# calclavia/tal-asrd

Hardware: AMD Instinct MI355X
Metric: audio frames/sec (16 kHz, 10 ms hop) end-to-end log-mel -> TDS encoder -> diarization head (higher is better)
Workload: dtype f32 (dense layers: 3 x f16 MFMA hi/lo split, f32 accumulate); 1 GPU; 1 x 3600 s 16 kHz clip per GPU, each a whole-episode B=1 call (BASELINE.json configs[2]; SDModel path of tal/baseline/reconcile.py:76-85: log-mel -> TDS 80-800-1120-1440 -> 128-d feat + argmax over 6008 speakers); weights=synthetic deterministic, audio_resident_in_hbm=True

## Files before the change

tal_asrd_amd/csrc/gemm_common.h:

```cpp
#pragma once
#include "common.h"

namespace tal {

constexpr int BK = 32;

template <int MODE, int NSUB>
__device__ __forceinline__ void gemm_epilogue(const GemmArgs& g, const f32x16 (&acc)[NSUB], float* lds, float* Y,
                                              const float* bias, const float* res, int64_t m0, int n0, int lane,
                                              int w, int wm, int wn) {
    const int64_t M = g.M;
    const int N = g.N;
    const int colb = lane & 31;
    const int rowb = 4 * (lane >> 5);
    const float alpha = g.alpha;
    const f32x4 zero4 = {0.f, 0.f, 0.f, 0.f};
    float amax = 0.f;
    constexpr int CW = 32 * NSUB;
    if (MODE == 4) {
        float bcol[NSUB];
#pragma unroll
        for (int j = 0; j < NSUB; ++j) {
            const int col = n0 + (wn * NSUB + j) * 32 + colb;
            bcol[j] = (bias && col < N) ? bias[col] : 0.f;
// ... 38 lines not shown
        const bool cols_full = n_base + CW <= N;
        const bool buf_ok = g.ldy < (1 << 21) && (MODE != 2 || g.ldres < (1 << 21));
        auto uptr = [](const float* p) {
            const uint64_t v = reinterpret_cast<uint64_t>(p);
            const uint32_t lo = __builtin_amdgcn_readfirstlane((uint32_t)v), hi = __builtin_amdgcn_readfirstlane((uint32_t)(v >> 32));
            return reinterpret_cast<void*>(((uint64_t)hi << 32) | lo);
        };
        __amdgpu_buffer_rsrc_t rs_y[2], rs_res[2];
#pragma unroll
        for (int half = 0; half < 2; ++half) {
            const int64_t row0 = m0 + wm * 32 + half * 16;
            const int rows_valid = (int)(M - row0 < 0 ? 0 : (M - row0 > 16 ? 16 : M - row0));
            const int ext_y = rows_valid > 0 ? (int)(((rows_valid - 1) * g.ldy + CW) * 4) : 0;
            const int ext_r = rows_valid > 0 && MODE == 2 ? (int)(((rows_valid - 1) * g.ldres + CW) * 4) : 0;
            rs_y[half] = __builtin_amdgcn_make_buffer_rsrc(uptr(Y + row0 * g.ldy + n_base), 0, __builtin_amdgcn_readfirstlane(ext_y), 0x00020000);
            rs_res[half] = __builtin_amdgcn_make_buffer_rsrc(uptr(MODE == 2 ? res + row0 * g.ldres + n_base : Y), 0,
                                                             __builtin_amdgcn_readfirstlane(ext_r), 0x00020000);
        }
        __amdgpu_buffer_rsrc_t rs_bias = __builtin_amdgcn_make_buffer_rsrc(uptr(bias ? bias + n_base : Y), 0, CW * 4, 0x00020000);
#pragma unroll
        for (int half = 0; half < 2; ++half) {
#pragma unroll
            for (int j = 0; j < NSUB; ++j)
#pragma unroll
                for (int e8 = 0; e8 < 8; ++e8) {
                    const int e = half * 8 + e8;
                    const int r = rowb + (e8 & 3) + 8 * (e8 >> 2);
                    stage[r * CW + j * 32 + colb] = acc[j][e];
                }
            if (cols_full && buf_ok) {
                typedef unsigned u32x4 __attribute__((ext_vector_type(4)));
                int r = lane / (CW / 4), c4 = lane - r * (CW / 4);
                int offy[2 * NSUB], offr[2 * NSUB], offb[2 * NSUB], ldsv[2 * NSUB];
                f32x4 rv[2 * NSUB], bv[2 * NSUB];
#pragma unroll
                for (int t = 0; t < 2 * NSUB; ++t) {
                    offy[t] = (r * (int)g.ldy + c4 * 4) * 4;
                    offr[t] = (r * (int)g.ldres + c4 * 4) * 4;
                    offb[t] = c4 * 16;
                    ldsv[t] = r * CW + c4 * 4;
                    c4 += 64 - CW / 4;
                    r += 1;
                    if (c4 >= CW / 4) {
                        c4 -= CW / 4;
                        r += 1;
                    }
                }
                typedef unsigned u32x2r __attribute__((ext_vector_type(2)));
                u32x2r rh[2 * NSUB], rl[2 * NSUB];
#pragma unroll
                for (int t = 0; t < 2 * NSUB; ++t) {
                    if (MODE == 2 && g.res_split) {
                        const int cw = offb[t] >> 2;
                        const int so = offr[t] - offb[t] + (cw >> 5) * 128 + (cw & 31) * 2;
                        rh[t] = __builtin_amdgcn_raw_buffer_load_b64(rs_res[half], so, 0, 0);
                        rl[t] = __builtin_amdgcn_raw_buffer_load_b64(rs_res[half], so + 64, 0, 0);
                    } else if (MODE == 2)
                        rv[t] = __builtin_bit_cast(f32x4, __builtin_amdgcn_raw_buffer_load_b128(rs_res[half], offr[t], 0, 0));
                    bv[t] = bias ? __builtin_bit_cast(f32x4, __builtin_amdgcn_raw_buffer_load_b128(rs_bias, offb[t], 0, 0)) : zero4;
                }
#pragma unroll
                for (int t = 0; t < 2 * NSUB; ++t) {
                    f32x4 v = *reinterpret_cast<const f32x4*>(&stage[ldsv[t]]) + bv[t];
                    if (MODE == 1) {
                        v.x = fmaxf(v.x, 0.f); v.y = fmaxf(v.y, 0.f); v.z = fmaxf(v.z, 0.f); v.w = fmaxf(v.w, 0.f);
                    }
                    if (MODE == 2 && g.res_split) {
                        const f16x4 h4 = __builtin_bit_cast(f16x4, rh[t]), l4 = __builtin_bit_cast(f16x4, rl[t]);
#pragma unroll
                        for (int q = 0; q < 4; ++q) rv[t][q] = (float)h4[q] + (float)l4[q] * (1.0f / 2048.0f);
                    }
                    if (MODE == 2) v = rv[t] + alpha * v;
                    if (MODE == 3 && (g.scale_cols == 0 || n_base + (offb[t] >> 2) < g.scale_cols)) v = alpha * v;
                    if (g.out_split) {
                        typedef unsigned u32x2 __attribute__((ext_vector_type(2)));
                        f16x4 hi, lo;
                        amax = amax4(amax, v);
                        if (g.range_flag) {
                            f16x2p h01, l01, h23, l23;
                            split_f16x3_pair(v.x, v.y, h01, l01);
                            split_f16x3_pair(v.z, v.w, h23, l23);
                            hi = {h01[0], h01[1], h23[0], h23[1]};
                            lo = {l01[0], l01[1], l23[0], l23[1]};
                        } else {
#pragma unroll
                            for (int q = 0; q < 4; ++q) {
                                _Float16 h, l;
                                split_f16x3(v[q], h, l);
                                hi[q] = h;
                                lo[q] = l;
                            }
                        }
                        const int cw = offb[t] >> 2;
                        const int so = offy[t] - offb[t] + (cw >> 5) * 128 + (cw & 31) * 2;
                        __builtin_amdgcn_raw_buffer_store_b64(__builtin_bit_cast(u32x2, hi), rs_y[half], so, 0, 0);
                        __builtin_amdgcn_raw_buffer_store_b64(__builtin_bit_cast(u32x2, lo), rs_y[half], so + 64, 0, 0);
                        continue;
                    }
                    __builtin_amdgcn_raw_buffer_store_b128(__builtin_bit_cast(u32x4, v), rs_y[half], offy[t], 0, 0);
                }
                if (g.out_split && half == 1) note_range(amax, g.range_flag);
                continue;
            }
#pragma unroll
            for (int t = 0; t < 2 * NSUB; ++t) {
                const int i = lane + 64 * t;
                const int r = i / (CW / 4);
                const int c = (i - r * (CW / 4)) * 4;
                const int64_t row = m0 + wm * 32 + half * 16 + r;
                const int col = n_base + c;
                if (row < M && col < N) {
                    f32x4 v = *reinterpret_cast<const f32x4*>(&stage[r * CW + c]);
                    if (col + 3 < N) {
                        if (bias) v += *reinterpret_cast<const f32x4*>(bias + col);
                        if (MODE == 1) {
                            v.x = fmaxf(v.x, 0.f); v.y = fmaxf(v.y, 0.f); v.z = fmaxf(v.z, 0.f); v.w = fmaxf(v.w, 0.f);
                        }
                        if (MODE == 2) v = *reinterpret_cast<const f32x4*>(res + row * g.ldres + col) + alpha * v;
                        if (MODE == 3 && (g.scale_cols == 0 || col < g.scale_cols)) v = alpha * v;
                        *reinterpret_cast<f32x4*>(Y + row * g.ldy + col) = v;
                    } else {
                        for (int q = 0; q < 4 && col + q < N; ++q) {
                            float x = v[q] + (bias ? bias[col + q] : 0.f);
                            if (MODE == 1) x = fmaxf(x, 0.f);
                            if (MODE == 2) x = res[row * g.ldres + col + q] + alpha * x;
                            if (MODE == 3 && (g.scale_cols == 0 || col + q < g.scale_cols)) x = alpha * x;
                            Y[row * g.ldy + col + q] = x;
                        }
                    }
                }
            }
        }
    } else {
#pragma unroll
        for (int j = 0; j < NSUB; ++j) {
            const int col = n0 + (wn * NSUB + j) * 32 + colb;
            if (col >= N) continue;
            const float bv = bias ? bias[col] : 0.f;
#pragma unroll
            for (int e = 0; e < 16; ++e) {
                const int64_t row = m0 + wm * 32 + rowb + (e & 3) + 8 * (e >> 2);
                if (row < M) {
                    float v = acc[j][e] + bv;
                    if (MODE == 1) v = fmaxf(v, 0.f);
                    if (MODE == 2) v = res[row * g.ldres + col] + alpha * v;
                    if (MODE == 3 && (g.scale_cols == 0 || col < g.scale_cols)) v = alpha * v;
                    Y[row * g.ldy + col] = v;
                }
            }
        }
    }
}

template <int MODE, int NSUB>
__device__ __forceinline__ void gemm_epilogue_split(const GemmArgs& g, const f32x16 (&acc)[NSUB], float* lds, float* Y,
                                                    const float* res, int64_t m0, int n0, int lane, int w) {
    static_assert(MODE == 1 || MODE == 2, "relu or residual");
    constexpr int CW = 32 * NSUB;
    typedef unsigned u32x2 __attribute__((ext_vector_type(2)));
    typedef float f32x2 __attribute__((ext_vector_type(2)));
    const int64_t M = g.M;
    const int colb = lane & 31, rowb = 4 * (lane >> 5);
    float* stage = lds + w * (16 * CW);
    auto uptr = [](const float* p) {
        const uint64_t v = reinterpret_cast<uint64_t>(p);
        const uint32_t lo = __builtin_amdgcn_readfirstlane((uint32_t)v), hi = __builtin_amdgcn_readfirstlane((uint32_t)(v >> 32));
        return reinterpret_cast<void*>(((uint64_t)hi << 32) | lo);
    };
    const int lr = lane >> 3, lp = lane & 7;
    const int ldy4 = (int)g.ldy * 4, ldr4 = (int)g.ldres * 4;
    const int vy0 = lr * ldy4 + lp * 8, vy1 = vy0 + 8 * ldy4;
    const int vr0 = lr * ldr4 + lp * 8, vr1 = vr0 + 8 * ldr4;
    const float* sp = stage + lr * CW + lp * 4;
    const float alpha = g.alpha;
    const f32x2 al2 = {alpha, alpha}, s11 = {1.0f / 2048.0f, 1.0f / 2048.0f};
    float amax = 0.f;
#pragma unroll
    for (int half = 0; half < 2; ++half) {
        const int64_t row0 = m0 + w * 32 + half * 16;
        const int rows_valid = (int)(M - row0 < 0 ? 0 : (M - row0 > 16 ? 16 : M - row0));
        const int ext_y = rows_valid > 0 ? (rows_valid - 1) * ldy4 + CW * 4 : 0;
        const int ext_r = rows_valid > 0 && MODE == 2 ? (rows_valid - 1) * ldr4 + CW * 4 : 0;
        __amdgpu_buffer_rsrc_t rs_y = __builtin_amdgcn_make_buffer_rsrc(uptr(Y + row0 * g.ldy + n0), 0, __builtin_amdgcn_readfirstlane(ext_y), 0x00020000);
        __amdgpu_buffer_rsrc_t rs_r = __builtin_amdgcn_make_buffer_rsrc(uptr(MODE == 2 ? res + row0 * g.ldres + n0 : Y), 0,
                                                                      __builtin_amdgcn_readfirstlane(ext_r), 0x00020000);
        u32x2 rh[2 * NSUB], rl[2 * NSUB];
        if (MODE == 2) {
#pragma unroll
            for (int t = 0; t < 2 * NSUB; ++t) {
                const int rg = t / NSUB, b = t % NSUB;
                rh[t] = __builtin_amdgcn_raw_buffer_load_b64(rs_r, (rg ? vr1 : vr0) + b * 128, 0, 0);
                rl[t] = __builtin_amdgcn_raw_buffer_load_b64(rs_r, (rg ? vr1 : vr0) + b * 128 + 64, 0, 0);
            }
        }
#pragma unroll
        for (int j = 0; j < NSUB; ++j)
#pragma unroll
            for (int e8 = 0; e8 < 8; ++e8) {
                const int r = rowb + (e8 & 3) + 8 * (e8 >> 2);
                stage[r * CW + j * 32 + colb] = acc[j][half * 8 + e8];
            }
        f32x4 sv[2 * NSUB];
#pragma unroll
        for (int t = 0; t < 2 * NSUB; ++t) sv[t] = *reinterpret_cast<const f32x4*>(sp + (t / NSUB) * 8 * CW + (t % NSUB) * 32);
#pragma unroll
        for (int t = 0; t < 2 * NSUB; ++t) {
            const int rg = t / NSUB, b = t % NSUB;
            f32x2 va = {sv[t][0], sv[t][1]}, vb = {sv[t][2], sv[t][3]};
            if (MODE == 1) {
                va = __builtin_elementwise_max(va, f32x2{0.f, 0.f});
                vb = __builtin_elementwise_max(vb, f32x2{0.f, 0.f});
            } else {
                const f16x4 h4 = __builtin_bit_cast(f16x4, rh[t]), l4 = __builtin_bit_cast(f16x4, rl[t]);
                const f32x2 ha = {(float)h4[0], (float)h4[1]}, hb = {(float)h4[2], (float)h4[3]};
                const f32x2 la = {(float)l4[0], (float)l4[1]}, lb = {(float)l4[2], (float)l4[3]};
                va = al2 * va + (la * s11 + ha);
                vb = al2 * vb + (lb * s11 + hb);
            }
            amax = __builtin_fmaxf(amax, __builtin_fmaxf(__builtin_fabsf(va[0]), __builtin_fabsf(va[1])));
            amax = __builtin_fmaxf(amax, __builtin_fmaxf(__builtin_fabsf(vb[0]), __builtin_fabsf(vb[1])));
            f16x2p h01, l01, h23, l23;
            split_f16x3_pair(va[0], va[1], h01, l01);
            split_f16x3_pair(vb[0], vb[1], h23, l23);
            const f16x4 hi = {h01[0], h01[1], h23[0], h23[1]}, lo = {l01[0], l01[1], l23[0], l23[1]};
            __builtin_amdgcn_raw_buffer_store_b64(__builtin_bit_cast(u32x2, hi), rs_y, (rg ? vy1 : vy0) + b * 128, 0, 0);
            __builtin_amdgcn_raw_buffer_store_b64(__builtin_bit_cast(u32x2, lo), rs_y, (rg ? vy1 : vy0) + b * 128 + 64, 0, 0);
        }
    }
    note_range(amax, g.range_flag);
}

__device__ __forceinline__ unsigned logical_tile_of(unsigned nb, unsigned bid) {
    const unsigned xcd = bid & 7u, q = nb >> 3, r = nb & 7u;
    return (xcd < r ? xcd * (q + 1) : r * (q + 1) + (xcd - r) * q) + (bid >> 3);
}
__device__ __forceinline__ unsigned logical_tile() { return logical_tile_of(gridDim.x, blockIdx.x); }

}
```

tal_asrd_amd/csrc/gemm_f32.hip:

```cpp
#include "gemm_common.h"

namespace tal {

template <int MODE, int NSUB, bool SPLITK, int STAGE, bool F16X3 = false, int EPI = 0>
__global__ __launch_bounds__(256, F16X3 ? 2 : 1) void gemm_glds_kernel(const GemmArgs g) {
    __builtin_amdgcn_s_setprio(3);
    constexpr int BM = 128, BN = 32 * NSUB;
    constexpr int ROWS = BM + BN;
    constexpr int CHUNKS = ROWS / 8;
    constexpr int PER_WAVE = CHUNKS / 4;
    __shared__ __attribute__((aligned(16))) float lds[2 * ROWS * 32];

    const bool is_slice = SPLITK && blockIdx.x >= (unsigned)g.tile_base;
    const unsigned sbid = blockIdx.x - (unsigned)g.tile_base;
    const int slice = is_slice ? (int)(sbid / (unsigned)g.tail_tiles) : 0;
    const unsigned logical = is_slice ? (unsigned)g.tile_base + sbid % (unsigned)g.tail_tiles
                                      : (SPLITK ? logical_tile_of((unsigned)g.tile_base, blockIdx.x) : logical_tile());
    const unsigned tile_m = g.tiles_n == 1 ? logical : __umulhi(logical, g.tiles_n_magic);
    const int64_t m0 = (int64_t)tile_m * BM;
    const int n0 = (int)(logical - tile_m * (unsigned)g.tiles_n) * BN;
    const int64_t M = g.M;
    const int N = g.N, K = g.K;
    const int z1 = EPI ? 0 : (int)blockIdx.y / g.nb2, z2 = EPI ? 0 : (int)blockIdx.y % g.nb2;
    const float* A = g.A + z1 * g.a_s1 + z2 * g.a_s2;
    const float* W = g.W + z1 * g.w_s1 + z2 * g.w_s2;
    float* Y = g.Y + z1 * g.y_s1 + z2 * g.y_s2;
    const float* bias = g.bias ? g.bias + z2 * g.bias_s2 : nullptr;
    const float* res = g.res ? g.res + z1 * g.r_s1 + z2 * g.r_s2 : nullptr;

    const int tid = threadIdx.x;
    const int lane = tid & 63;
    const int w = wave_id();
    const int wm = w, wn = 0;

    const int sub = lane >> 3;
    const int srccol = ((lane & 7) ^ (((w & 1) * 4 + (lane >> 4)) & 7)) * 4;
    const int a_rows = (int)((M - m0) < BM ? (M - m0) : BM) - 1;
    const int b_rows = ((N - n0) < BN ? (N - n0) : BN) - 1;
    const float* src[PER_WAVE];
#pragma unroll
    for (int t = 0; t < PER_WAVE; ++t) {
        const int row = 8 * (w + 4 * t) + sub;
        if (t < 4)
            src[t] = A + (m0 + min(row, a_rows)) * g.lda + srccol;
        else
            src[t] = W + (int64_t)(n0 + min(row - BM, b_rows)) * g.ldw + srccol;
    }
    auto uniform_ptr = [](const float* p) {
        const uint64_t v = reinterpret_cast<uint64_t>(p);
        const uint32_t lo = __builtin_amdgcn_readfirstlane((uint32_t)v), hi = __builtin_amdgcn_readfirstlane((uint32_t)(v >> 32));
        return reinterpret_cast<void*>(((uint64_t)hi << 32) | lo);
    };
    __amdgpu_buffer_rsrc_t rsrc_a = __builtin_amdgcn_make_buffer_rsrc(uniform_ptr(A + m0 * g.lda), 0, 0x7fffffff, 0x00020000);
    __amdgpu_buffer_rsrc_t rsrc_w = __builtin_amdgcn_make_buffer_rsrc(uniform_ptr(W + (int64_t)n0 * g.ldw), 0, 0x7fffffff, 0x00020000);
    int voff[PER_WAVE];
#pragma unroll
    for (int t = 0; t < PER_WAVE; ++t) {
        const int row = 8 * (w + 4 * t) + sub;
        voff[t] = t < 4 ? (int)((min(row, a_rows) * g.lda + srccol) * 4) : (int)((min(row - BM, b_rows) * g.ldw + srccol) * 4);
    }
    auto issue = [&](int kt, int buf) {
#pragma unroll
        for (int t = 0; t < PER_WAVE; ++t) {
            float* dst = lds + buf * (ROWS * 32) + (w + 4 * t) * 256;
            if (STAGE == 2) {
#if defined(__HIP_DEVICE_COMPILE__)
                __builtin_amdgcn_raw_ptr_buffer_load_lds(t < 4 ? rsrc_a : rsrc_w, (__attribute__((address_space(3))) void*)dst, 16,
                                                         voff[t], kt * (BK * 4), 0, 0);
#endif
            } else
                __builtin_amdgcn_global_load_lds((const __attribute__((address_space(1))) void*)(src[t] + kt * BK),
                                                 (__attribute__((address_space(3))) void*)dst, 16, 0, 0);
        }
    };

    f32x16 acc[NSUB];
    f32x16 accx[F16X3 ? NSUB : 1];
#pragma unroll
    for (int j = 0; j < NSUB; ++j) {
        const float b0 = (EPI && bias && !is_slice) ? bias[n0 + j * 32 + (lane & 31)] : 0.f;
#pragma unroll
        for (int e = 0; e < 16; ++e) acc[j][e] = b0;
    }
#pragma unroll
    for (int j = 0; j < (F16X3 ? NSUB : 1); ++j)
#pragma unroll
        for (int e = 0; e < 16; ++e) accx[j][e] = 0.f;

    const int frow = lane & 31;
    const int fsw = (frow >> 1) & 7;
    const int fhalf = lane >> 5;
    const int nk_all = K / BK;
    const int kt0 = is_slice ? (int)((int64_t)slice * nk_all / g.split) : 0;
    const int nk = is_slice ? (int)((int64_t)(slice + 1) * nk_all / g.split) : nk_all;
    issue(kt0, kt0 & 1);
    __builtin_amdgcn_s_setprio(0);
    __builtin_assume(kt0 < nk);
    for (int kt = kt0; kt < nk; ++kt) {
        asm volatile("s_waitcnt vmcnt(0)" ::: "memory");
        __syncthreads();
        if (kt + 1 < nk) issue(kt + 1, (kt + 1) & 1);
        const float* As = lds + (kt & 1) * (ROWS * 32) + (wm * 32 + frow) * 32;
        const float* Bs = lds + (kt & 1) * (ROWS * 32) + (BM + frow) * 32;
        if (F16X3) {
            f16x8 ahi[2], alo[2], bhi[3], blo[3];
            auto slh = [&](int gk) { return ((2 * gk + fhalf) ^ fsw) * 4; };
            auto sll = [&](int gk) { return ((4 + 2 * gk + fhalf) ^ fsw) * 4; };
            auto read_b = [&](int q, int slot) {
                const int gk = q / NSUB, j = q % NSUB;
                bhi[slot] = *reinterpret_cast<const f16x8*>(Bs + j * 32 * 32 + slh(gk));
                blo[slot] = *reinterpret_cast<const f16x8*>(Bs + j * 32 * 32 + sll(gk));
            };
            ahi[0] = *reinterpret_cast<const f16x8*>(As + slh(0));
            alo[0] = *reinterpret_cast<const f16x8*>(As + sll(0));
            read_b(0, 0);
            read_b(1, 1);
#pragma unroll
            for (int q = 0; q < 2 * NSUB; ++q) {
                const int gk = q / NSUB, j = q % NSUB;
                if (q + 2 < 2 * NSUB) read_b(q + 2, (q + 2) % 3);
                if (q == NSUB - 2) {
                    ahi[1] = *reinterpret_cast<const f16x8*>(As + slh(1));
                    alo[1] = *reinterpret_cast<const f16x8*>(As + sll(1));
                }
                __builtin_amdgcn_sched_barrier(0);
                acc[j] = __builtin_amdgcn_mfma_f32_32x32x16_f16(ahi[gk], bhi[q % 3], acc[j], 0, 0, 0);
                accx[F16X3 ? j : 0] = __builtin_amdgcn_mfma_f32_32x32x16_f16(ahi[gk], blo[q % 3], accx[F16X3 ? j : 0], 0, 0, 0);
                accx[F16X3 ? j : 0] = __builtin_amdgcn_mfma_f32_32x32x16_f16(alo[gk], bhi[q % 3], accx[F16X3 ? j : 0], 0, 0, 0);
                __builtin_amdgcn_sched_barrier(0);
            }
            continue;
        }
        f32x4 fa[2], fb[2][NSUB];
        fa[0] = *reinterpret_cast<const f32x4*>(As + ((fhalf) ^ fsw) * 4);
#pragma unroll
        for (int j = 0; j < NSUB; ++j) fb[0][j] = *reinterpret_cast<const f32x4*>(Bs + j * 32 * 32 + ((fhalf) ^ fsw) * 4);
#pragma unroll
        for (int kk = 0; kk < BK / 8; ++kk) {
            const int cur = kk & 1, nxt = cur ^ 1;
            if (kk + 1 < BK / 8) {
                const int sl = ((2 * (kk + 1) + fhalf) ^ fsw) * 4;
                fa[nxt] = *reinterpret_cast<const f32x4*>(As + sl);
#pragma unroll
                for (int j = 0; j < NSUB; ++j) fb[nxt][j] = *reinterpret_cast<const f32x4*>(Bs + j * 32 * 32 + sl);
            }
#pragma unroll
            for (int j = 0; j < NSUB; ++j) {
                acc[j] = __builtin_amdgcn_mfma_f32_32x32x2f32(fa[cur].x, fb[cur][j].x, acc[j], 0, 0, 0);
                acc[j] = __builtin_amdgcn_mfma_f32_32x32x2f32(fa[cur].y, fb[cur][j].y, acc[j], 0, 0, 0);
                acc[j] = __builtin_amdgcn_mfma_f32_32x32x2f32(fa[cur].z, fb[cur][j].z, acc[j], 0, 0, 0);
                acc[j] = __builtin_amdgcn_mfma_f32_32x32x2f32(fa[cur].w, fb[cur][j].w, acc[j], 0, 0, 0);
            }
        }
    }
    asm volatile("s_waitcnt vmcnt(0)" ::: "memory");
    __syncthreads();
    __builtin_amdgcn_s_setprio(3);
    if (F16X3) {
        typedef float f32x2 __attribute__((ext_vector_type(2)));
        const f32x2 s11 = {1.0f / 2048.0f, 1.0f / 2048.0f};
#pragma unroll
        for (int j = 0; j < NSUB; ++j)
#pragma unroll
            for (int e = 0; e < 16; e += 2) {
                const f32x2 x2 = {accx[F16X3 ? j : 0][e], accx[F16X3 ? j : 0][e + 1]}, a2 = {acc[j][e], acc[j][e + 1]};
                const f32x2 o2 = __builtin_elementwise_fma(x2, s11, a2);
                acc[j][e] = o2[0];
                acc[j][e + 1] = o2[1];
            }
    }
    if (is_slice) {
        GemmArgs gp = g;
        gp.M = m0 + BM;
        gp.N = n0 + BN;
        gp.ldy = BN;
        gp.out_split = 0;
        float* tile_ws = g.splitk_ws + ((size_t)(logical - g.tile_base) * g.split + slice) * (BM * BN);
        gemm_epilogue<0, NSUB>(gp, acc, lds, tile_ws - (m0 * BN + n0), nullptr, nullptr, m0, n0, lane, w, wm, wn);
    } else {
        if constexpr (EPI != 0) gemm_epilogue_split<MODE, NSUB>(g, acc, lds, Y, res, m0, n0, lane, w);
        else gemm_epilogue<MODE, NSUB>(g, acc, lds, Y, bias, res, m0, n0, lane, w, wm, wn);
    }
}

template <int MODE, int WAVES_M, int NSUB, int BKT>
__global__ __launch_bounds__(256) void gemm_nt_f32_kernel(const GemmArgs g) {
    constexpr int WAVES_N = 4 / WAVES_M;
    constexpr int BM = 32 * WAVES_M;
    constexpr int BN = 32 * NSUB * WAVES_N;
    constexpr int LDS_LD = BKT + 4;
    constexpr int C4 = BKT / 4;
    constexpr int RPP = 256 / C4;
    constexpr int A_LOADS = BM / RPP;
    constexpr int B_LOADS = BN / RPP;
    __shared__ __attribute__((aligned(16))) float lds[(BM + BN) * LDS_LD];
    float* As = lds;
    float* Bs = lds + BM * LDS_LD;

    const unsigned logical = logical_tile();
    const int64_t m0 = (int64_t)(logical / (unsigned)g.tiles_n) * BM;
    const int n0 = (int)(logical % (unsigned)g.tiles_n) * BN;
    const int64_t M = g.M;
    const int N = g.N, K = g.K;

    const int z1 = (int)blockIdx.y / g.nb2, z2 = (int)blockIdx.y % g.nb2;
    const float* A = g.A + z1 * g.a_s1 + z2 * g.a_s2;
    const float* W = g.W + z1 * g.w_s1 + z2 * g.w_s2;
    float* Y = g.Y + z1 * g.y_s1 + z2 * g.y_s2;
    const float* bias = g.bias ? g.bias + z2 * g.bias_s2 : nullptr;
    const float* res = g.res ? g.res + z1 * g.r_s1 + z2 * g.r_s2 : nullptr;

    const int tid = threadIdx.x;
    const int lane = tid & 63;
    const int w = wave_id();
    const int wm = w / WAVES_N, wn = w % WAVES_N;
    const int lrow = tid / C4;
    const int lc4 = tid % C4;

    const float* At = A + m0 * g.lda + lc4 * 4;
    const float* Wt = W + (int64_t)n0 * g.ldw + lc4 * 4;
    const int a_rows = (int)((M - m0) < BM ? (M - m0) : BM) - 1;
    const int b_rows = ((N - n0) < BN ? (N - n0) : BN) - 1;
    int64_t a_off[A_LOADS], b_off[B_LOADS];
#pragma unroll
    for (int p = 0; p < A_LOADS; ++p) a_off[p] = min(lrow + RPP * p, a_rows) * g.lda;
#pragma unroll
    for (int p = 0; p < B_LOADS; ++p) b_off[p] = min(lrow + RPP * p, b_rows) * g.ldw;

    f32x16 acc[NSUB];
#pragma unroll
    for (int j = 0; j < NSUB; ++j)
#pragma unroll
        for (int e = 0; e < 16; ++e) acc[j][e] = 0.f;

    const f32x4 zero4 = {0.f, 0.f, 0.f, 0.f};
    f32x4 ra[A_LOADS], rb[B_LOADS];
    bool in_cur = lc4 * 4 < K;
    {
        const int ko = in_cur ? 0 : -lc4 * 4;
#pragma unroll
        for (int p = 0; p < A_LOADS; ++p) ra[p] = *reinterpret_cast<const f32x4*>(At + ko + a_off[p]);
#pragma unroll
        for (int p = 0; p < B_LOADS; ++p) rb[p] = *reinterpret_cast<const f32x4*>(Wt + ko + b_off[p]);
    }

    const int frag_off = (lane & 31) * LDS_LD + (lane >> 5) * 4;
    const int nk = (K + BKT - 1) / BKT;
    for (int kt = 0; kt < nk; ++kt) {
#pragma unroll
        for (int p = 0; p < A_LOADS; ++p)
            *reinterpret_cast<f32x4*>(&As[(lrow + RPP * p) * LDS_LD + lc4 * 4]) = in_cur ? ra[p] : zero4;
#pragma unroll
        for (int p = 0; p < B_LOADS; ++p)
            *reinterpret_cast<f32x4*>(&Bs[(lrow + RPP * p) * LDS_LD + lc4 * 4]) = in_cur ? rb[p] : zero4;
        __syncthreads();
        if (kt + 1 < nk) {
            in_cur = (kt + 1) * BKT + lc4 * 4 < K;
            const int ko = in_cur ? (kt + 1) * BKT : -lc4 * 4;
#pragma unroll
            for (int p = 0; p < A_LOADS; ++p) ra[p] = *reinterpret_cast<const f32x4*>(At + ko + a_off[p]);
#pragma unroll
            for (int p = 0; p < B_LOADS; ++p) rb[p] = *reinterpret_cast<const f32x4*>(Wt + ko + b_off[p]);
        }
        f32x4 fa[2], fb[2][NSUB];
        fa[0] = *reinterpret_cast<const f32x4*>(&As[wm * 32 * LDS_LD + frag_off]);
#pragma unroll
        for (int j = 0; j < NSUB; ++j)
            fb[0][j] = *reinterpret_cast<const f32x4*>(&Bs[(wn * NSUB + j) * 32 * LDS_LD + frag_off]);
#pragma unroll
        for (int kk = 0; kk < BKT / 8; ++kk) {
            const int cur = kk & 1, nxt = cur ^ 1;
            if (kk + 1 < BKT / 8) {
                fa[nxt] = *reinterpret_cast<const f32x4*>(&As[wm * 32 * LDS_LD + frag_off + (kk + 1) * 8]);
#pragma unroll
                for (int j = 0; j < NSUB; ++j)
                    fb[nxt][j] = *reinterpret_cast<const f32x4*>(
                        &Bs[(wn * NSUB + j) * 32 * LDS_LD + frag_off + (kk + 1) * 8]);
            }
#pragma unroll
            for (int j = 0; j < NSUB; ++j) {
                acc[j] = __builtin_amdgcn_mfma_f32_32x32x2f32(fa[cur].x, fb[cur][j].x, acc[j], 0, 0, 0);
                acc[j] = __builtin_amdgcn_mfma_f32_32x32x2f32(fa[cur].y, fb[cur][j].y, acc[j], 0, 0, 0);
                acc[j] = __builtin_amdgcn_mfma_f32_32x32x2f32(fa[cur].z, fb[cur][j].z, acc[j], 0, 0, 0);
                acc[j] = __builtin_amdgcn_mfma_f32_32x32x2f32(fa[cur].w, fb[cur][j].w, acc[j], 0, 0, 0);
            }
        }
        __syncthreads();
    }
    gemm_epilogue<MODE, NSUB>(g, acc, lds, Y, bias, res, m0, n0, lane, w, wm, wn);
}

template <int WAVES_M, int NSUB, int BKT>
static void launch_tile(const GemmArgs& g, int mode, dim3 grid, hipStream_t s) {
    switch (mode) {
        case 0: hipLaunchKernelGGL((gemm_nt_f32_kernel<0, WAVES_M, NSUB, BKT>), grid, dim3(256), 0, s, g); break;
        case 1: hipLaunchKernelGGL((gemm_nt_f32_kernel<1, WAVES_M, NSUB, BKT>), grid, dim3(256), 0, s, g); break;
        case 2: hipLaunchKernelGGL((gemm_nt_f32_kernel<2, WAVES_M, NSUB, BKT>), grid, dim3(256), 0, s, g); break;
        case 3: hipLaunchKernelGGL((gemm_nt_f32_kernel<3, WAVES_M, NSUB, BKT>), grid, dim3(256), 0, s, g); break;
        default: hipLaunchKernelGGL((gemm_nt_f32_kernel<4, WAVES_M, NSUB, BKT>), grid, dim3(256), 0, s, g); break;
    }
}

template <int MODE, int NW>
__global__ __launch_bounds__(64 * NW) void gemm_splitk4_kernel(const GemmArgs g) {
    constexpr int PITCH = 68;
    constexpr int SLAB = 32 * PITCH;
    __shared__ __attribute__((aligned(16))) float smem[NW * 2 * SLAB];
    float* part = smem;
    const int tiles_n = g.tiles_n;
    const int64_t m0 = (int64_t)(blockIdx.x / (unsigned)tiles_n) * 32;
    const int n0 = (int)(blockIdx.x % (unsigned)tiles_n) * 32;
    const int64_t M = g.M;
    const int N = g.N, K = g.K;
    const int z1 = (int)blockIdx.y / g.nb2, z2 = (int)blockIdx.y % g.nb2;
    const float* A = g.A + z1 * g.a_s1 + z2 * g.a_s2;
    const float* W = g.W + z1 * g.w_s1 + z2 * g.w_s2;
    float* Y = g.Y + z1 * g.y_s1 + z2 * g.y_s2;
    const float* bias = g.bias ? g.bias + z2 * g.bias_s2 : nullptr;
    const float* res = g.res ? g.res + z1 * g.r_s1 + z2 * g.r_s2 : nullptr;

    const int tid = threadIdx.x, lane = tid & 63, w = wave_id();
    const int r32 = lane & 31, kh = lane >> 5;
    const int lrow = lane >> 4, lcol = (lane & 15) * 4;
    const float* aptr[8];
    const float* wptr[8];
#pragma unroll
    for (int j = 0; j < 8; ++j) {
        const int64_t ar = m0 + 4 * j + lrow;
        const int wr = n0 + 4 * j + lrow;
        aptr[j] = A + (ar < M ? ar : M - 1) * g.lda + lcol;
        wptr[j] = W + (int64_t)(wr < N ? wr : N - 1) * g.ldw + lcol;
    }
    float* As = smem + w * (2 * SLAB);
    float* Ws = As + SLAB;
// ... 434 lines not shown
```

tal_asrd_amd/csrc/gemm_w64.hip:

```cpp
#include <type_traits>

#include "gemm_common.h"

namespace tal {

namespace {

typedef unsigned u32x4w __attribute__((ext_vector_type(4)));

constexpr int W_BM = 256, W_NSUB = 5, W_BN = 32 * W_NSUB, W_ROWS = W_BM + W_BN, W_NBUF = 3;
constexpr int W_CHUNKS = W_ROWS / 8, W_PER_WAVE = W_CHUNKS / 4, W_AT = W_BM / 8 / 4;
constexpr int W_BUF_FLOATS = W_ROWS * 32;
static_assert(W_CHUNKS % 4 == 0, "chunks divide over the waves");

constexpr int dma_piece(int q, int slot) { return (slot < 2 && q < 6) ? 2 * q + slot : (q == 6 && slot == 0) ? 12 : -1; }

__device__ __forceinline__ void mfma_vgpr(f32x16& c, const f16x8& a, const f16x8& b) {
    asm volatile("v_mfma_f32_32x32x16_f16 %0, %1, %2, %0" : "+v"(c) : "v"(a), "v"(b));
}
#define W64_MFMA(c, a, b, in_vgpr) do { if (in_vgpr) mfma_vgpr(c, a, b); else c = __builtin_amdgcn_mfma_f32_32x32x16_f16(a, b, c, 0, 0, 0); } while (0)

struct Frags {
    f16x8 ahi[2][2], alo[2][2];
    f16x8 bhi[5], blo[5];
};

}

template <int MODE, bool SPLITK, int EPI>
__global__ __launch_bounds__(256, 1) void gemm_w64_kernel(const GemmArgs g) {
    constexpr int NSUB = W_NSUB, BM = W_BM, BN = W_BN, PER_WAVE = W_PER_WAVE, A_T = W_AT, BUF_FLOATS = W_BUF_FLOATS;
    __shared__ __attribute__((aligned(16))) float lds[W_NBUF * W_BUF_FLOATS];

    if (g.stagger_ticks > 0 && blockIdx.x < (unsigned)g.stagger_blocks && (blockIdx.x & 1u)) {
        const unsigned long long t0 = wall_clock64();
        while (wall_clock64() - t0 < (unsigned long long)g.stagger_ticks) __builtin_amdgcn_s_sleep(64);
    }
    const bool is_slice = SPLITK && blockIdx.x >= (unsigned)g.tile_base;
    const unsigned sbid = blockIdx.x - (unsigned)g.tile_base;
    const int slice = is_slice ? (int)(sbid / (unsigned)g.tail_tiles) : 0;
    const unsigned logical = is_slice ? (unsigned)g.tile_base + sbid % (unsigned)g.tail_tiles
                                      : (SPLITK ? logical_tile_of((unsigned)g.tile_base, blockIdx.x) : logical_tile());
    const unsigned tile_m = g.tiles_n == 1 ? logical : __umulhi(logical, g.tiles_n_magic);
    const int64_t m0 = (int64_t)tile_m * BM;
    const int n0 = (int)(logical - tile_m * (unsigned)g.tiles_n) * BN;
    const int64_t M = g.M;
    const int N = g.N, K = g.K;
    const float* A = g.A;
    const float* W = g.W;
    const int tid = threadIdx.x, lane = tid & 63;
    const int w = wave_id();

    const int sub = lane >> 3, srccol = ((lane & 7) ^ (((w & 1) * 4 + (lane >> 4)) & 7)) * 4;
    const int a_rows = (int)((M - m0) < BM ? (M - m0) : BM) - 1;
    const int b_rows = ((N - n0) < BN ? (N - n0) : BN) - 1;
    auto make_rsrc = [](const float* p) {
        const uint64_t v = reinterpret_cast<uint64_t>(p);
        u32x4w r;
        r[0] = __builtin_amdgcn_readfirstlane((uint32_t)v);
        r[1] = __builtin_amdgcn_readfirstlane((uint32_t)(v >> 32));
        r[2] = 0x7fffffffu;
        r[3] = 0x00020000u;
        return r;
    };
    const u32x4w rs_a = make_rsrc(A + m0 * g.lda), rs_w = make_rsrc(W + (int64_t)n0 * g.ldw);
    const unsigned lds_base = __builtin_amdgcn_readfirstlane((unsigned)(size_t)(__attribute__((address_space(3))) float*)lds) + (unsigned)w * 1024u;
    int voff[PER_WAVE];
#pragma unroll
    for (int t = 0; t < PER_WAVE; ++t) {
        const int row = 8 * (w + 4 * t) + sub;
        voff[t] = t < A_T ? (int)((min(row, a_rows) * g.lda + srccol) * 4) : (int)((min(row - BM, b_rows) * g.ldw + srccol) * 4);
    }
    auto dma = [&](int t, unsigned nrec, int bufoff, int kofs) {
        const unsigned dst = lds_base + (unsigned)(bufoff * 4 + t * 4096);
        u32x4w rs = t < A_T ? rs_a : rs_w;
        rs[2] = nrec;
        asm volatile("s_mov_b32 m0, %0\n\ts_nop 0\n\tbuffer_load_dwordx4 %1, %2, %3 offen lds" ::"s"(dst), "v"(voff[t]), "s"(rs), "s"(kofs) : "memory");
    };

    f32x16 hh[2][NSUB], xx[2][NSUB];
#pragma unroll
    for (int j = 0; j < NSUB; ++j) {
        const float b0 = (EPI && g.bias && !is_slice) ? g.bias[n0 + j * 32 + (lane & 31)] : 0.f;
#pragma unroll
        for (int b = 0; b < 2; ++b)
#pragma unroll
            for (int e = 0; e < 16; ++e) {
                hh[b][j][e] = b0;
                xx[b][j][e] = 0.f;
            }
    }

    const int frow = lane & 31, fsw = (frow >> 1) & 7, fhalf = lane >> 5, fc = fhalf ^ fsw;
    const int a_lane = (w * 64 + frow) * 32, b_lane = (BM + frow) * 32;
    auto slot = [&](int x) { return (x ^ fc) * 4; };
    Frags f;
    auto read_a = [&](int gk, int bufoff) {
#pragma unroll
        for (int b = 0; b < 2; ++b) {
            f.ahi[gk][b] = *reinterpret_cast<const f16x8*>(lds + bufoff + a_lane + b * 32 * 32 + slot(2 * gk));
            f.alo[gk][b] = *reinterpret_cast<const f16x8*>(lds + bufoff + a_lane + b * 32 * 32 + slot(4 + 2 * gk));
        }
    };
    auto rb = [&](int q, int bufoff) {
        const int gk = q / NSUB, j = q % NSUB;
        f.bhi[j] = *reinterpret_cast<const f16x8*>(lds + bufoff + b_lane + j * 32 * 32 + slot(2 * gk));
        f.blo[j] = *reinterpret_cast<const f16x8*>(lds + bufoff + b_lane + j * 32 * 32 + slot(4 + 2 * gk));
    };

    const int nk_all = K / BK;
    const int kt0 = is_slice ? (int)((int64_t)slice * nk_all / g.split) : 0;
    const int kt1 = is_slice ? (int)((int64_t)(slice + 1) * nk_all / g.split) : nk_all;
    constexpr unsigned NREC = 0x7fffffffu;
#pragma unroll
    for (int t = 0; t < PER_WAVE; ++t) dma(t, NREC, 0, kt0 * (BK * 4));
    {
        const unsigned nrec = kt0 + 1 < kt1 ? NREC : 0u;
#pragma unroll
        for (int t = 0; t < PER_WAVE; ++t) dma(t, nrec, BUF_FLOATS, (kt0 + 1) * (BK * 4));
    }
    asm volatile("s_waitcnt vmcnt(%0)" ::"n"(PER_WAVE) : "memory");
    __builtin_amdgcn_s_barrier();
    read_a(0, 0);
    rb(0, 0);
    rb(1, 0);
    auto step = [&](auto bufc, int kt) {
        constexpr int cur = decltype(bufc)::value * BUF_FLOATS, nxt = ((decltype(bufc)::value + 1) % 3) * BUF_FLOATS,
                      fil = ((decltype(bufc)::value + 2) % 3) * BUF_FLOATS;
        const int kofs = (kt + 2) * (BK * 4);
        const unsigned nrec = kt + 2 < kt1 ? NREC : 0u;
#pragma unroll
        for (int q = 0; q < 2 * NSUB; ++q) {
            const int gk = q / NSUB, j = q % NSUB;
            if (q == 8) {
                asm volatile("s_waitcnt vmcnt(%0)" ::"n"(PER_WAVE) : "memory");
                __builtin_amdgcn_s_barrier();
            }
            if (q + 2 < 2 * NSUB) rb(q + 2, cur);
            else rb(q + 2 - 2 * NSUB, nxt);
            if (q == 8) read_a(0, nxt);
            if (q == 2) read_a(1, cur);
            __builtin_amdgcn_sched_barrier(0);
            const bool vg = j >= 3, vx0 = j >= 4;
            W64_MFMA(hh[0][j], f.ahi[gk][0], f.bhi[j], false);
            W64_MFMA(hh[1][j], f.ahi[gk][1], f.bhi[j], vg);
            if (dma_piece(q, 0) >= 0) { __builtin_amdgcn_sched_barrier(0); dma(dma_piece(q, 0), nrec, fil, kofs); __builtin_amdgcn_sched_barrier(0); }
            W64_MFMA(xx[0][j], f.ahi[gk][0], f.blo[j], vx0);
            W64_MFMA(xx[1][j], f.ahi[gk][1], f.blo[j], vg);
            if (dma_piece(q, 1) >= 0) { __builtin_amdgcn_sched_barrier(0); dma(dma_piece(q, 1), nrec, fil, kofs); __builtin_amdgcn_sched_barrier(0); }
            W64_MFMA(xx[0][j], f.alo[gk][0], f.bhi[j], vx0);
            W64_MFMA(xx[1][j], f.alo[gk][1], f.bhi[j], vg);
            if (dma_piece(q, 2) >= 0) { __builtin_amdgcn_sched_barrier(0); dma(dma_piece(q, 2), nrec, fil, kofs); }
            __builtin_amdgcn_sched_barrier(0);
        }
    };
    int kt = kt0;
    for (; kt + 3 <= kt1; kt += 3) {
        step(std::integral_constant<int, 0>(), kt);
        step(std::integral_constant<int, 1>(), kt + 1);
        step(std::integral_constant<int, 2>(), kt + 2);
    }
    if (kt < kt1) step(std::integral_constant<int, 0>(), kt);
    if (kt + 1 < kt1) step(std::integral_constant<int, 1>(), kt + 1);
    asm volatile("s_waitcnt vmcnt(0)\n\ts_nop 15\n\ts_nop 15" ::: "memory");
    __syncthreads();

    typedef float f32x2 __attribute__((ext_vector_type(2)));
    const f32x2 s11 = {1.0f / 2048.0f, 1.0f / 2048.0f};
    auto finish = [&](auto bc) {
        constexpr int b = decltype(bc)::value;
        f32x16 acc[NSUB];
#pragma unroll
        for (int j = 0; j < NSUB; ++j)
#pragma unroll
            for (int e = 0; e < 16; e += 2) {
                const f32x2 x2 = {xx[b][j][e], xx[b][j][e + 1]}, a2 = {hh[b][j][e], hh[b][j][e + 1]};
                const f32x2 o2 = __builtin_elementwise_fma(x2, s11, a2);
                acc[j][e] = o2[0];
                acc[j][e + 1] = o2[1];
            }
        const int64_t m0e = m0 + 32 * w + 32 * b;
        if (b == 1) __builtin_amdgcn_wave_barrier();
        if (is_slice) {
            GemmArgs gp = g;
            gp.M = m0 + BM;
            gp.N = n0 + BN;
            gp.ldy = BN;
            gp.out_split = 0;
            float* tile_ws = g.splitk_ws + ((size_t)(logical - g.tile_base) * g.split + slice) * (BM * BN);
            gemm_epilogue<0, NSUB>(gp, acc, lds, tile_ws - (m0 * BN + n0), nullptr, nullptr, m0e, n0, lane, w, w, 0);
        } else {
            if constexpr (EPI != 0) gemm_epilogue_split<MODE, NSUB>(g, acc, lds, g.Y, g.res, m0e, n0, lane, w);
            else gemm_epilogue<MODE, NSUB>(g, acc, lds, g.Y, g.bias, g.res, m0e, n0, lane, w, w, 0);
        }
    };
    finish(std::integral_constant<int, 0>());
    finish(std::integral_constant<int, 1>());
}

template <int MODE, bool SPLITK>
static void launch_w64_mode(const GemmArgs& g, dim3 grid, hipStream_t s) {
    if constexpr (MODE == 1 || MODE == 2) {
        const bool y_ok = g.ldy % 4 == 0 && g.ldy < (1 << 21) && (reinterpret_cast<uintptr_t>(g.Y) & 15) == 0 && g.N % W_BN == 0;
        const bool r_ok = MODE != 2 || (g.res_split && g.ldres % 4 == 0 && g.ldres < (1 << 21) && (reinterpret_cast<uintptr_t>(g.res) & 15) == 0);
        if (g.out_split && g.range_flag && y_ok && r_ok) {
            hipLaunchKernelGGL((gemm_w64_kernel<MODE, SPLITK, 1>), grid, dim3(256), 0, s, g);
            return;
        }
    }
    hipLaunchKernelGGL((gemm_w64_kernel<MODE, SPLITK, 0>), grid, dim3(256), 0, s, g);
}

void launch_gemm_w64(const GemmArgs& g0, int mode, bool splitk, dim3 grid, hipStream_t s) {
    GemmArgs g = g0;
    const int pct = opt(OPT_GEMM_W64_STAGGER);
    if (pct > 0 && grid.x >= 2u * (unsigned)device_cus()) {
        const double tile_us = 1.39 * (g.K / 32) + 12.0;
        g.stagger_ticks = (int)(tile_us * pct);
        g.stagger_blocks = device_cus();
    }
    if (splitk) {
        switch (mode) {
            case 0: launch_w64_mode<0, true>(g, grid, s); break;
            case 1: launch_w64_mode<1, true>(g, grid, s); break;
            case 2: launch_w64_mode<2, true>(g, grid, s); break;
            default: launch_w64_mode<3, true>(g, grid, s); break;
        }
        return;
    }
    switch (mode) {
        case 0: launch_w64_mode<0, false>(g, grid, s); break;
        case 1: launch_w64_mode<1, false>(g, grid, s); break;
        case 2: launch_w64_mode<2, false>(g, grid, s); break;
        default: launch_w64_mode<3, false>(g, grid, s); break;
    }
}

}
```

Before: 21.58 million frames/s.

## Prefetch residual tiles early and widen split-epilogue loads and stores to 128-bit

The residual hi/lo fp16 tiles for the split epilogue are now requested before the accumulator finalisation. Each half's epilogue issues the load for the next 16-row slab, so global latency overlaps the LDS staging and conversion work. Loads and stores move from 64-bit to 128-bit buffer operations with a new lane mapping. An XOR swizzle on the staging writes is meant to avoid LDS bank conflicts. The range amax is carried across both finish calls and reported once. In exchange, the prefetched residual values are held in registers longer, which raises register pressure.

```diff
diff --git a/tal_asrd_amd/csrc/gemm_common.h b/tal_asrd_amd/csrc/gemm_common.h
--- a/tal_asrd_amd/csrc/gemm_common.h
+++ b/tal_asrd_amd/csrc/gemm_common.h
@@ -214,82 +214,106 @@
     }
 }
 
-template <int MODE, int NSUB>
+typedef unsigned u32x4e __attribute__((ext_vector_type(4)));
+template <int NSUB>
+struct SplitResidual {
+    u32x4e h[NSUB], l[NSUB];
+};
+
+__device__ __forceinline__ __amdgpu_buffer_rsrc_t gemm_split_window(const float* p, int64_t row0, int64_t M, int ld4, int width4) {
+    const uint64_t v = reinterpret_cast<uint64_t>(p);
+    const uint32_t lo = __builtin_amdgcn_readfirstlane((uint32_t)v), hi = __builtin_amdgcn_readfirstlane((uint32_t)(v >> 32));
+    const int rows_valid = (int)(M - row0 < 0 ? 0 : (M - row0 > 16 ? 16 : M - row0));
+    const int ext = rows_valid > 0 ? (rows_valid - 1) * ld4 + width4 : 0;
+    return __builtin_amdgcn_make_buffer_rsrc(reinterpret_cast<void*>(((uint64_t)hi << 32) | lo), 0, __builtin_amdgcn_readfirstlane(ext), 0x00020000);
+}
+
+template <int NSUB>
+__device__ __forceinline__ void gemm_split_residual_request(const GemmArgs& g, const float* res, int64_t row0, int n0, int lane,
+                                                            SplitResidual<NSUB>& r) {
+    const int ldr4 = (int)g.ldres * 4;
+    const int vr = (lane >> 2) * ldr4 + (lane & 3) * 16;
+    __amdgpu_buffer_rsrc_t rs = gemm_split_window(res + row0 * g.ldres + n0, row0, g.M, ldr4, NSUB * 128);
+#pragma unroll
+    for (int b = 0; b < NSUB; ++b) {
+        r.h[b] = __builtin_amdgcn_raw_buffer_load_b128(rs, vr + b * 128, 0, 0);
+        r.l[b] = __builtin_amdgcn_raw_buffer_load_b128(rs, vr + b * 128 + 64, 0, 0);
+    }
+}
+
+template <int MODE, int NSUB, bool LAST>
 __device__ __forceinline__ void gemm_epilogue_split(const GemmArgs& g, const f32x16 (&acc)[NSUB], float* lds, float* Y,
-                                                    const float* res, int64_t m0, int n0, int lane, int w) {
+                                                    const float* res, int64_t m0, int n0, int lane, int w,
+                                                    SplitResidual<NSUB>& rcur, float& amax) {
     static_assert(MODE == 1 || MODE == 2, "relu or residual");
     constexpr int CW = 32 * NSUB;
-    typedef unsigned u32x2 __attribute__((ext_vector_type(2)));
     typedef float f32x2 __attribute__((ext_vector_type(2)));
-    const int64_t M = g.M;
+    typedef _Float16 f16x8e __attribute__((ext_vector_type(8)));
     const int colb = lane & 31, rowb = 4 * (lane >> 5);
     float* stage = lds + w * (16 * CW);
-    auto uptr = [](const float* p) {
-        const uint64_t v = reinterpret_cast<uint64_t>(p);
-        const uint32_t lo = __builtin_amdgcn_readfirstlane((uint32_t)v), hi = __builtin_amdgcn_readfirstlane((uint32_t)(v >> 32));
-        return reinterpret_cast<void*>(((uint64_t)hi << 32) | lo);
-    };
-    const int lr = lane >> 3, lp = lane & 7;
-    const int ldy4 = (int)g.ldy * 4, ldr4 = (int)g.ldres * 4;
-    const int vy0 = lr * ldy4 + lp * 8, vy1 = vy0 + 8 * ldy4;
-    const int vr0 = lr * ldr4 + lp * 8, vr1 = vr0 + 8 * ldr4;
-    const float* sp = stage + lr * CW + lp * 4;
+    float* wp0 = stage + rowb * CW + colb;
+    float* wp1 = stage + rowb * CW + (colb ^ 4);
+    const int lr = lane >> 2, lp = lane & 3, ls = (lr >> 1) & 1;
+    const int ldy4 = (int)g.ldy * 4;
+    const int vy = lr * ldy4 + lp * 16;
+    const float* sp0 = stage + lr * CW + lp * 8 + 4 * ls;
+    const float* sp1 = stage + lr * CW + lp * 8 + 4 * (1 - ls);
     const float alpha = g.alpha;
     const f32x2 al2 = {alpha, alpha}, s11 = {1.0f / 2048.0f, 1.0f / 2048.0f};
-    float amax = 0.f;
 #pragma unroll
     for (int half = 0; half < 2; ++half) {
         const int64_t row0 = m0 + w * 32 + half * 16;
-        const int rows_valid = (int)(M - row0 < 0 ? 0 : (M - row0 > 16 ? 16 : M - row0));
-        const int ext_y = rows_valid > 0 ? (rows_valid - 1) * ldy4 + CW * 4 : 0;
-        const int ext_r = rows_valid > 0 && MODE == 2 ? (rows_valid - 1) * ldr4 + CW * 4 : 0;
-        __amdgpu_buffer_rsrc_t rs_y = __builtin_amdgcn_make_buffer_rsrc(uptr(Y + row0 * g.ldy + n0), 0, __builtin_amdgcn_readfirstlane(ext_y), 0x00020000);
-        __amdgpu_buffer_rsrc_t rs_r = __builtin_amdgcn_make_buffer_rsrc(uptr(MODE == 2 ? res + row0 * g.ldres + n0 : Y), 0,
-                                                                      __builtin_amdgcn_readfirstlane(ext_r), 0x00020000);
-        u32x2 rh[2 * NSUB], rl[2 * NSUB];
-        if (MODE == 2) {
-#pragma unroll
-            for (int t = 0; t < 2 * NSUB; ++t) {
-                const int rg = t / NSUB, b = t % NSUB;
-                rh[t] = __builtin_amdgcn_raw_buffer_load_b64(rs_r, (rg ? vr1 : vr0) + b * 128, 0, 0);
-                rl[t] = __builtin_amdgcn_raw_buffer_load_b64(rs_r, (rg ? vr1 : vr0) + b * 128 + 64, 0, 0);
-            }
-        }
+        SplitResidual<NSUB> rnext;
+        if (MODE == 2 && (half == 0 || !LAST)) gemm_split_residual_request<NSUB>(g, res, row0 + 16, n0, lane, rnext);
+        __amdgpu_buffer_rsrc_t rs_y = gemm_split_window(Y + row0 * g.ldy + n0, row0, g.M, ldy4, CW * 4);
 #pragma unroll
         for (int j = 0; j < NSUB; ++j)
 #pragma unroll
             for (int e8 = 0; e8 < 8; ++e8) {
-                const int r = rowb + (e8 & 3) + 8 * (e8 >> 2);
-                stage[r * CW + j * 32 + colb] = acc[j][half * 8 + e8];
-            }
-        f32x4 sv[2 * NSUB];
-#pragma unroll
-        for (int t = 0; t < 2 * NSUB; ++t) sv[t] = *reinterpret_cast<const f32x4*>(sp + (t / NSUB) * 8 * CW + (t % NSUB) * 32);
-#pragma unroll
-        for (int t = 0; t < 2 * NSUB; ++t) {
-            const int rg = t / NSUB, b = t % NSUB;
-            f32x2 va = {sv[t][0], sv[t][1]}, vb = {sv[t][2], sv[t][3]};
-            if (MODE == 1) {
-                va = __builtin_elementwise_max(va, f32x2{0.f, 0.f});
-                vb = __builtin_elementwise_max(vb, f32x2{0.f, 0.f});
-            } else {
-                const f16x4 h4 = __builtin_bit_cast(f16x4, rh[t]), l4 = __builtin_bit_cast(f16x4, rl[t]);
-                const f32x2 ha = {(float)h4[0], (float)h4[1]}, hb = {(float)h4[2], (float)h4[3]};
-                const f32x2 la = {(float)l4[0], (float)l4[1]}, lb = {(float)l4[2], (float)l4[3]};
-                va = al2 * va + (la * s11 + ha);
-                vb = al2 * vb + (lb * s11 + hb);
-            }
-            amax = __builtin_fmaxf(amax, __builtin_fmaxf(__builtin_fabsf(va[0]), __builtin_fabsf(va[1])));
-            amax = __builtin_fmaxf(amax, __builtin_fmaxf(__builtin_fabsf(vb[0]), __builtin_fabsf(vb[1])));
-            f16x2p h01, l01, h23, l23;
-            split_f16x3_pair(va[0], va[1], h01, l01);
-            split_f16x3_pair(vb[0], vb[1], h23, l23);
-            const f16x4 hi = {h01[0], h01[1], h23[0], h23[1]}, lo = {l01[0], l01[1], l23[0], l23[1]};
-            __builtin_amdgcn_raw_buffer_store_b64(__builtin_bit_cast(u32x2, hi), rs_y, (rg ? vy1 : vy0) + b * 128, 0, 0);
-            __builtin_amdgcn_raw_buffer_store_b64(__builtin_bit_cast(u32x2, lo), rs_y, (rg ? vy1 : vy0) + b * 128 + 64, 0, 0);
-        }
+                const int r = (e8 & 3) + 8 * (e8 >> 2);
+                ((e8 & 2) ? wp1 : wp0)[r * CW + j * 32] = acc[j][half * 8 + e8];
+            }
+        f32x4 sa[2 * NSUB];
+#pragma unroll
+        for (int b = 0; b < NSUB; ++b) {
+            sa[2 * b] = *reinterpret_cast<const f32x4*>(sp0 + b * 32);
+            sa[2 * b + 1] = *reinterpret_cast<const f32x4*>(sp1 + b * 32);
+        }
+        __builtin_amdgcn_sched_barrier(0);
+#pragma unroll
+        for (int b = 0; b < NSUB; ++b) {
+            const f32x4 sv[2] = {sa[2 * b], sa[2 * b + 1]};
+            f16x8e h8, l8, hi, lo;
+            if (MODE == 2) {
+                h8 = __builtin_bit_cast(f16x8e, rcur.h[b]);
+                l8 = __builtin_bit_cast(f16x8e, rcur.l[b]);
+            }
+#pragma unroll
+            for (int q = 0; q < 2; ++q) {
+                f32x2 va = {sv[q][0], sv[q][1]}, vb = {sv[q][2], sv[q][3]};
+                if (MODE == 1) {
+                    va = __builtin_elementwise_max(va, f32x2{0.f, 0.f});
+                    vb = __builtin_elementwise_max(vb, f32x2{0.f, 0.f});
+                } else {
+                    const f32x2 ha = {(float)h8[4 * q], (float)h8[4 * q + 1]}, hb = {(float)h8[4 * q + 2], (float)h8[4 * q + 3]};
+                    const f32x2 la = {(float)l8[4 * q], (float)l8[4 * q + 1]}, lb = {(float)l8[4 * q + 2], (float)l8[4 * q + 3]};
+                    va = al2 * va + (la * s11 + ha);
+                    vb = al2 * vb + (lb * s11 + hb);
+                }
+                amax = __builtin_fmaxf(amax, __builtin_fmaxf(__builtin_fabsf(va[0]), __builtin_fabsf(va[1])));
+                amax = __builtin_fmaxf(amax, __builtin_fmaxf(__builtin_fabsf(vb[0]), __builtin_fabsf(vb[1])));
+                f16x2p h01, l01, h23, l23;
+                split_f16x3_pair(va[0], va[1], h01, l01);
+                split_f16x3_pair(vb[0], vb[1], h23, l23);
+                hi[4 * q] = h01[0]; hi[4 * q + 1] = h01[1]; hi[4 * q + 2] = h23[0]; hi[4 * q + 3] = h23[1];
+                lo[4 * q] = l01[0]; lo[4 * q + 1] = l01[1]; lo[4 * q + 2] = l23[0]; lo[4 * q + 3] = l23[1];
+            }
+            __builtin_amdgcn_raw_buffer_store_b128(__builtin_bit_cast(u32x4e, hi), rs_y, vy + b * 128, 0, 0);
+            __builtin_amdgcn_raw_buffer_store_b128(__builtin_bit_cast(u32x4e, lo), rs_y, vy + b * 128 + 64, 0, 0);
+        }
+        if (MODE == 2 && (half == 0 || !LAST)) rcur = rnext;
     }
-    note_range(amax, g.range_flag);
+    if (LAST) note_range(amax, g.range_flag);
 }
 
 __device__ __forceinline__ unsigned logical_tile_of(unsigned nb, unsigned bid) {
diff --git a/tal_asrd_amd/csrc/gemm_f32.hip b/tal_asrd_amd/csrc/gemm_f32.hip
--- a/tal_asrd_amd/csrc/gemm_f32.hip
+++ b/tal_asrd_amd/csrc/gemm_f32.hip
@@ -156,6 +156,9 @@
     asm volatile("s_waitcnt vmcnt(0)" ::: "memory");
     __syncthreads();
     __builtin_amdgcn_s_setprio(3);
+    SplitResidual<NSUB> rres;
+    if constexpr (EPI != 0 && MODE == 2)
+        if (!is_slice) gemm_split_residual_request<NSUB>(g, res, m0 + 32 * w, n0, lane, rres);
     if (F16X3) {
         typedef float f32x2 __attribute__((ext_vector_type(2)));
         const f32x2 s11 = {1.0f / 2048.0f, 1.0f / 2048.0f};
@@ -178,8 +181,11 @@
         float* tile_ws = g.splitk_ws + ((size_t)(logical - g.tile_base) * g.split + slice) * (BM * BN);
         gemm_epilogue<0, NSUB>(gp, acc, lds, tile_ws - (m0 * BN + n0), nullptr, nullptr, m0, n0, lane, w, wm, wn);
     } else {
-        if constexpr (EPI != 0) gemm_epilogue_split<MODE, NSUB>(g, acc, lds, Y, res, m0, n0, lane, w);
-        else gemm_epilogue<MODE, NSUB>(g, acc, lds, Y, bias, res, m0, n0, lane, w, wm, wn);
+        if constexpr (EPI != 0) {
+            float amax = 0.f;
+            gemm_epilogue_split<MODE, NSUB, true>(g, acc, lds, Y, res, m0, n0, lane, w, rres, amax);
+        } else
+            gemm_epilogue<MODE, NSUB>(g, acc, lds, Y, bias, res, m0, n0, lane, w, wm, wn);
     }
 }
 
diff --git a/tal_asrd_amd/csrc/gemm_w64.hip b/tal_asrd_amd/csrc/gemm_w64.hip
--- a/tal_asrd_amd/csrc/gemm_w64.hip
+++ b/tal_asrd_amd/csrc/gemm_w64.hip
@@ -167,6 +167,8 @@
 
     typedef float f32x2 __attribute__((ext_vector_type(2)));
     const f32x2 s11 = {1.0f / 2048.0f, 1.0f / 2048.0f};
+    SplitResidual<NSUB> rres;
+    float amax = 0.f;
     auto finish = [&](auto bc) {
         constexpr int b = decltype(bc)::value;
         f32x16 acc[NSUB];
@@ -190,10 +192,12 @@
             float* tile_ws = g.splitk_ws + ((size_t)(logical - g.tile_base) * g.split + slice) * (BM * BN);
             gemm_epilogue<0, NSUB>(gp, acc, lds, tile_ws - (m0 * BN + n0), nullptr, nullptr, m0e, n0, lane, w, w, 0);
         } else {
-            if constexpr (EPI != 0) gemm_epilogue_split<MODE, NSUB>(g, acc, lds, g.Y, g.res, m0e, n0, lane, w);
+            if constexpr (EPI != 0) gemm_epilogue_split<MODE, NSUB, b == 1>(g, acc, lds, g.Y, g.res, m0e, n0, lane, w, rres, amax);
             else gemm_epilogue<MODE, NSUB>(g, acc, lds, g.Y, g.bias, g.res, m0e, n0, lane, w, w, 0);
         }
     };
+    if constexpr (EPI != 0 && MODE == 2)
+        if (!is_slice) gemm_split_residual_request<NSUB>(g, g.res, m0 + 64 * w, n0, lane, rres);
     finish(std::integral_constant<int, 0>());
     finish(std::integral_constant<int, 1>());
 }
```

Measured after the change: 21.71 million frames/s (median of 6 runs). Within noise of the previous version (+0.6%).
